# YuvalNirkin/hyperseg

Measured on AMD Instinct MI355X. Metric: frames/sec @ bs=1 HyperSeg-M 1024x512, higher is better.
Workload: dtype f32 storage and accumulation; level-4 inverted residual products as 3-term f16 splits (f32-class: 1.3e-7 of sum|a||b|; exact_f32 beside it)

## Files before the change

### hyperseg_amd/_hip.py

```python
import ctypes as C
import os
import types

import torch

_LIB_PATH = os.environ.get('HS_HIP_LIB') or os.path.join(os.path.dirname(os.path.abspath(__file__)), 'lib',
                                                         'libhyperseg_hip.so')

ACT_NONE, ACT_RELU, ACT_RELU6, ACT_SWISH = 0, 1, 2, 3
PAD_MODES = {'zeros': 0, 'reflect': 1, 'replicate': 2, 'circular': 3}
PREV_NONE, PREV_SAME, PREV_BILINEAR = 0, 1, 2

_STATUS = {-1: 'bad argument', -2: 'feature map does not tile into the weight grid (H % fh or W % fw != 0)',
           -3: 'unsupported shape', -4: 'tile does not fit the LDS'}


class HipLibraryError(RuntimeError):
    pass


class StageInputC(C.Structure):
    _fields_ = [('skip', C.c_void_p), ('prev', C.c_void_p),
                ('batch', C.c_int32), ('H', C.c_int32), ('W', C.c_int32),
                ('c_skip', C.c_int32), ('c_prev', C.c_int32),
# ... 15 lines not shown
    _fields_ = [('skip', C.c_void_p), ('c_skip', C.c_int32), ('bank', C.c_void_p), ('ld', C.c_int64), ('c_out', C.c_int32),
                ('scale', C.c_void_p), ('shift', C.c_void_p), ('act', C.c_int32)]


class SeTailC(C.Structure):
    _fields_ = [('w_reduce', C.c_void_p), ('b_reduce', C.c_void_p), ('w_expand_t', C.c_void_p), ('b_expand', C.c_void_p), ('c_squeezed', C.c_int32),
                ('gate', C.c_void_p), ('squeezed', C.c_void_p), ('workspace', C.c_void_p)]


class ChainIrLevelC(C.Structure):
    _fields_ = [('skip', C.c_void_p), ('c_skip', C.c_int32), ('bank', C.c_void_p), ('ld', C.c_int64), ('hidden', C.c_int32), ('c_out', C.c_int32),
                ('s1', C.c_void_p), ('b1', C.c_void_p), ('s2', C.c_void_p), ('b2', C.c_void_p), ('s3', C.c_void_p), ('b3', C.c_void_p)]


class S2wTrainLayerC(C.Structure):
    _fields_ = [('signal_index', C.c_int32), ('signal_channels', C.c_int32), ('groups', C.c_int32),
                ('w', C.c_void_p), ('wc', C.c_int32), ('rows', C.c_int32),
                ('bank', C.c_void_p), ('ld', C.c_int64), ('dbank', C.c_void_p), ('dw', C.c_void_p), ('ds', C.c_void_p)]


class TtaPassC(C.Structure):
    _fields_ = [('x', C.c_void_p), ('Hi', C.c_int32), ('Wi', C.c_int32), ('Hm', C.c_int32), ('Wm', C.c_int32),
                ('flipped', C.c_int32), ('entry', C.c_int32)]


STATUS = 'hs_status'
i32, i64, vp = C.c_int32, C.c_int64, C.c_void_p
SIGNATURES = {
    'hs_version': ([], C.c_int),
    'hs_build_info': ([], C.c_char_p),
    'hs_signal2weights_fwd': ([vp, i32, i32, i32, i32, i32, i32, i32, vp, i32, i32, vp, i64, vp], STATUS),
    'hs_signal2weights_multi_fwd': ([vp, i32, i32, i32, i32, C.POINTER(S2wLayerC), i32, vp], STATUS),
    'hs_s2w_pack_floats': ([i32, i32, i32], C.c_int64),
    'hs_s2w_pack_fwd': ([vp, i32, i32, i32, vp, vp], STATUS),
    'hs_bank_pack_fwd': ([vp, i32, i32, i32, i32, i32, i32, vp, i64, vp], STATUS),
    'hs_bn_fold_fwd': ([vp, vp, vp, vp, C.c_float, i32, vp, vp, vp], STATUS),
    'hs_patch_conv_fwd': ([C.POINTER(StageInputC), i32, i32, vp, i64, i32, i32, i32, i32, i32,
                           C.POINTER(EpilogueC), vp, vp], STATUS),
    'hs_patch_conv_s2w_fwd': ([C.POINTER(StageInputC), i32, i32, vp, i64, i32, i32, C.POINTER(EpilogueC), vp,
                               vp, i32, i32, i32, i32, C.POINTER(S2wLayerC), i32, vp], STATUS),
    'hs_k1_chain_workspace': ([i32, i32, i32, C.POINTER(K1LevelC), i32], C.c_int64),
    'hs_k1_chain_fwd': ([i32, i32, i32, C.POINTER(K1LevelC), i32, vp, vp, vp], STATUS),
    'hs_decoder_chain_workspace': ([i32, i32, i32, C.POINTER(K1LevelC), i32, C.POINTER(ChainIrLevelC)], C.c_int64),
    'hs_decoder_chain_fwd': ([i32, i32, i32, C.POINTER(K1LevelC), i32, C.POINTER(ChainIrLevelC), vp, vp, vp], STATUS),
    'hs_meta_conv_fwd': ([vp, i32, i32, i32, i32, vp, i64] + [i32] * 13 + [C.POINTER(EpilogueC), vp, vp], STATUS),
    'hs_meta_conv_bwd': ([vp, i32, i32, i32, i32, vp, i64] + [i32] * 12 + [vp, vp, vp, i64, vp], STATUS),
# ... 102 lines not shown
    'hs_label_resize_fwd': ([vp, i32, i32, i32, i32, vp, i32, vp, i32, i32, i32, i32, i32, i32, i32, vp, i32, vp], STATUS),
    'hs_resize_tables_fwd': ([vp, i32, i32, i32, i32, i32, i32, i32, vp, vp, vp, vp, vp], STATUS),
    'hs_frame_resize_batch_fwd': ([vp, i32, i32, i32, i32, vp, vp, vp, vp, i32, i32, i32, C.c_uint32, vp, vp, vp], STATUS),
    'hs_label_resize_batch_fwd': ([vp, i32, i32, i32, i32, vp, vp, vp, i32, i32, i32, vp, i32, vp], STATUS),
    'hs_label_encode_fwd': ([vp, i32, i32, i32, i32, vp, i32, i32, i32, vp, i32, vp], STATUS),
    'hs_label_resize_coded_fwd': ([vp, i32, i32, i32, i32, vp, i32, vp, i32, i32, i32, i32, i32, i32, i32, vp, i32, i32, i32, vp, i32, vp], STATUS),
    'hs_label_resize_batch_coded_fwd': ([vp, i32, i32, i32, i32, vp, vp, vp, i32, i32, i32, vp, i32, i32, i32, vp, i32, vp], STATUS),
    'hs_color_jitter_fwd': ([vp, i32, i32, i32, i32, vp, vp, vp, vp, vp], STATUS),
    'hs_gaussian_blur_fwd': ([vp, i32, i32, i32, i32, vp, vp, vp, vp, vp, vp], STATUS),
    'hs_frame_rotate_fwd': ([vp, i32, i32, i32, i32, vp, i32, i32, C.c_uint32, C.c_uint32, vp, vp, vp], STATUS),
    'hs_label_rotate_fwd': ([vp, i32, i32, i32, i32, vp, i32, i32, i32, i32, vp, i32, vp], STATUS),
    'hs_resize_tables_ragged_fwd': ([vp, i32, i32, i32, i32, i32, i32, i32, vp, vp, vp, vp, vp], STATUS),
    'hs_color_jitter_ragged_fwd': ([vp, i32, i32, i32, i32, vp, vp, vp, vp, vp], STATUS),
    'hs_frame_resize_ragged_fwd': ([vp, i32, i32, i32, i32, vp, vp, vp, vp, i32, i32, i32, vp, vp], STATUS),
    'hs_label_resize_ragged_fwd': ([vp, i32, i32, i32, i32, vp, vp, vp, i32, i32, vp, vp], STATUS),
    'hs_frame_rotate_ragged_fwd': ([vp, i32, i32, i32, i32, vp, vp, vp, i32, i32, C.c_uint32, C.c_uint32, vp, vp, vp], STATUS),
    'hs_label_rotate_ragged_fwd': ([vp, i32, i32, i32, vp, vp, vp, i32, i32, i32, i32, vp, i32, vp], STATUS),
    'hs_mbconv_expand_dw_fwd': ([vp, i32, i32, i32, i32, vp, i32, vp, vp, vp, i32, i32, i32, i32, i32, i32, vp, vp, vp, vp, vp], STATUS),
    'hs_se_gate_fwd': ([vp, i32, i32, i32, C.c_float, vp, vp, i32, vp, vp, vp, vp, vp, i32, vp, vp, vp], STATUS),
    'hs_gemm_split_kp': ([i32], C.c_int),
    'hs_gemm_split_fwd': ([vp, vp, vp, vp, vp, i32, vp, vp, i32, i32, i32, i32, i32, vp], STATUS),
    'hs_gemm_split_se_fwd': ([vp, vp, vp, i32, C.c_float, vp, vp, i32, vp, vp, vp, vp, i32, vp, vp, i32, i32, i32, i32, i32, vp, vp, vp], STATUS),
    'hs_gemm_split_se_route': ([i32] * 6, C.c_int),
    'hs_gemm_split_conv2x2_fwd': ([vp, vp, vp, vp, i32, vp, vp, i32, i32, i32, i32, i32, i32, vp], STATUS),
    'hs_gemm_split_up2_fwd': ([vp, vp, vp, vp, i32, vp, i32, i32, i32, i32, i32, i32, vp], STATUS),
    'hs_depthwise_route': ([i32] * 11, C.c_int),
    'hs_mbconv_route': ([i32] * 11, C.c_int),
    'hs_stem_dw_route': ([i32] * 9, C.c_int),
    'hs_stem_route': ([i32] * 3, C.c_int),
    'hs_se_gate_route': ([i32] * 5, C.c_int),
    'hs_pointwise_route': ([i32] * 5, C.c_int),
    'hs_pooled_shift_fwd': ([vp, i32, C.c_float, vp, vp, vp, i32, i32, vp], STATUS),
}
EXPORTS = list(SIGNATURES)


def check(status, what):
    if status == 0:
        return
    if status < 0:
        raise HipLibraryError(f'{what}: {_STATUS.get(status, status)}')
    raise HipLibraryError(f'{what}: HIP launch failed with hipError_t {status}')


def _raise_unless_ok(status, fn, args):
    if status:
# ... 65 lines not shown
```

### hyperseg_amd/csrc/hs_gemm_split.hip

```cpp
#include "hs_common.h"
#include "hs_se_gate_phases.h"
#include <type_traits>

namespace hs {

using half8 = __attribute__((ext_vector_type(8))) _Float16;
using gs_f32x4 = __attribute__((ext_vector_type(4))) float;

__device__ __forceinline__ int gs_exp_of(float m) { return min(max(__float_as_int(m) >> 23, 27), 254); }
__device__ __forceinline__ float gs_scale_of(int eb) { return __int_as_float((268 - eb) << 23); }
__device__ __forceinline__ float gs_inv_scale_of(int eb) { return __int_as_float((eb - 14) << 23); }

struct GemmSplitArgs {
    const _Float16* __restrict__ wf;
    const float* __restrict__ w_inv;
    const float* __restrict__ gate; const float* __restrict__ x;
    const float* shift;
    const float* residual;
    float* y;
    int M, K, KST, N, act;
    int conv_wo;
    float* pool_partial;
    int up2_wo;
};

struct GemmSeArgs {
    const float* __restrict__ partial;
    const float* __restrict__ w1; const float* __restrict__ b1;
    const float* __restrict__ w2t; const float* __restrict__ b2;
    float* gate_out; float* squeezed_out;
    float inv_hw; int nblk, Csq;
};
template <bool SEG> struct GemmSeOperand {};
template <> struct GemmSeOperand<true> : GemmSeArgs {};

#ifndef HS_GS_NARROW_MAX_WG
#define HS_GS_NARROW_MAX_WG 128
#endif

#ifndef HS_GS_TALL_MIN_WG
#define HS_GS_TALL_MIN_WG 257
#endif

template <int KS, int NWV, bool FAST, int NS, int MT, int NCH, bool PATCH, bool SEG = false>
__global__ __launch_bounds__(64 * NWV)
void gemm_split_kernel(GemmSplitArgs a, GemmSeOperand<SEG> se) {
    static_assert(!SEG || (FAST && !PATCH && NCH == 1 && (NWV == 8 ? KS <= 3 : KS == 1)), "SEG: the project convolutions' forms only");
    extern __shared__ __attribute__((aligned(16))) float gs_red[];
    constexpr int nthr = 64 * NWV, nwv = NWV;
    constexpr int NP = 16 * NS, NR = 16 * MT, NE = NR * NP;
    const int tid = threadIdx.x, lane = tid & 63, wave = tid >> 6;
    const int lrow = lane & 15, kg = lane >> 4;
    const int n0 = blockIdx.x * NP, r0 = blockIdx.y * MT, b = blockIdx.z;
    const float* __restrict__ xb = a.x + (size_t)b * a.K * a.N;
    const float* __restrict__ gb = a.gate ? a.gate + (size_t)b * a.K : nullptr;
    float* yb = a.y + (size_t)b * a.M * a.N * (a.up2_wo > 0 ? 4 : 1);
    const float* rb = a.residual ? a.residual + (size_t)b * a.M * a.N : nullptr;
    const int rt_max = (a.M + 15) >> 4;

    using gs_f32x2 = __attribute__((ext_vector_type(2))) float;
    const int ncol0 = min(n0 + NS * lrow, a.N - (FAST && !PATCH && NS == 2 ? 2 : 1)), ncol1 = min(n0 + NS * lrow + 1, a.N - 1);
    float xv[NCH][NS][KS][8];
    if constexpr (PATCH) {
        const int oy = ncol0 / a.conv_wo, ox = ncol0 - oy * a.conv_wo;
        const float* __restrict__ win = xb + (size_t)(2 * oy) * (2 * a.conv_wo) + 2 * ox;
        const int cmax = (a.K >> 2) - 1;
#pragma unroll
        for (int c = 0; c < NCH; ++c)
#pragma unroll
            for (int s = 0; s < KS; ++s)
#pragma unroll
                for (int q = 0; q < 4; ++q) {
                    const int ch = min((((wave * NCH + c) * KS + s) * 32 + 8 * kg) / 4 + (q >> 1), cmax);
                    const float* src = win + (size_t)ch * (4 * a.N) + (q & 1) * (2 * a.conv_wo);
                    if constexpr (NS == 1) {
                        const gs_f32x2 v = *reinterpret_cast<const gs_f32x2*>(src);
// ... 375 lines not shown
    GemmSeOperand<true> se{{partial, w_reduce, b_reduce, w_expand_t, b_expand, gate_out, squeezed_out, inv_hw, nblk, c_squeezed}};
    const size_t se_lds = (size_t)SEP_LDS_FLOATS * sizeof(float);
    const size_t lds = pol.lds > se_lds ? pol.lds : se_lds;
    hipStream_t s = (hipStream_t)stream;
#define HS_GSE(KSV, NWV) do { \
        if (pol.narrow) hipLaunchKernelGGL((gemm_split_kernel<KSV, NWV, true, 1, 2, 1, false, true>), pol.grid, dim3(64 * NWV), lds, s, a, se); \
        else if (pol.tall) hipLaunchKernelGGL((gemm_split_kernel<KSV, NWV, true, 2, 4, 1, false, true>), pol.grid, dim3(64 * NWV), lds, s, a, se); \
        else hipLaunchKernelGGL((gemm_split_kernel<KSV, NWV, true, 2, 2, 1, false, true>), pol.grid, dim3(64 * NWV), lds, s, a, se); } while (0)
    switch (pol.ks) {
        case 1: if (pol.nwv == 2) HS_GSE(1, 2); else if (pol.nwv == 4) HS_GSE(1, 4); else HS_GSE(1, 8); break;
        case 2: HS_GSE(2, 8); break;
        default: HS_GSE(3, 8); break;
    }
#undef HS_GSE
    return launch_status();
}

extern "C" int hs_gemm_split_fwd(const void* w_frag, const float* w_inv, const float* gate, const float* x,
                                 const float* shift, int32_t act, const float* residual, float* y,
                                 int32_t batch, int32_t c_out, int32_t c_in, int32_t kp, int32_t pixels, void* stream) {
    return launch_gemm_split_plain(w_frag, w_inv, gate, x, shift, act, residual, y, batch, c_out, c_in, kp, pixels, 0, stream);
}

extern "C" int hs_gemm_split_up2_fwd(const void* w_frag, const float* w_inv, const float* x, const float* shift, int32_t act,
                                     float* y, int32_t batch, int32_t c_out, int32_t c_in, int32_t kp, int32_t Ho, int32_t Wo,
                                     void* stream) {
    if (Ho <= 0 || Wo <= 0 || (((size_t)y) & 7) != 0) return HS_ERR_BAD_ARG;
    return launch_gemm_split_plain(w_frag, w_inv, nullptr, x, shift, act, nullptr, y, batch, c_out, c_in, kp, Ho * Wo, Wo, stream);
}

extern "C" int hs_pooled_shift_fwd(const float* partial, int32_t nblk, float inv_pixels, const float* wb, const float* shift,
                                   float* shift_out, int32_t rows, int32_t channels, void* stream) {
    if (!partial || !wb || !shift || !shift_out || nblk <= 0 || rows <= 0 || channels <= 0) return HS_ERR_BAD_ARG;
    if (channels > 8192) return HS_ERR_UNSUPPORTED;
    hipLaunchKernelGGL(pooled_shift_kernel, dim3((rows + 15) / 16), dim3(256), (size_t)channels * sizeof(float), (hipStream_t)stream,
                       partial, nblk, inv_pixels, wb, shift, shift_out, rows, channels);
    return launch_status();
}

extern "C" int hs_gemm_split_conv2x2_fwd(const void* w_frag, const float* w_inv, const float* x, const float* shift, int32_t act,
                                         float* y, float* pool_partial, int32_t batch, int32_t c_out, int32_t c_in, int32_t kp,
                                         int32_t Ho, int32_t Wo, void* stream) {
    if (!w_frag || !w_inv || !x || !y || batch <= 0 || c_out <= 0 || c_in <= 0 || Ho <= 0 || Wo <= 0) return HS_ERR_BAD_ARG;
    if (act < 0 || act > 3) return HS_ERR_BAD_ARG;
    int nwv, ks, nch;
    if (c_in > (1 << 20) || !gemm_split_plan(4 * c_in, nwv, ks, nch) || nwv != 8 || (Wo & 1) || (c_in & 1)) return HS_ERR_UNSUPPORTED;
// ... 24 lines not shown
```

### hyperseg_amd/functional.py

```python
import collections
import ctypes as C
import functools
import os
import threading

import torch

from . import _hip
from ._hip import ACT_NONE, ACT_RELU, ACT_RELU6, PAD_MODES

BN_EPS_DEFAULT = 1e-5
DTYPE_CODES = {torch.float32: 0, torch.bfloat16: 1, torch.float16: 2}
S2W_TRAIN_MAX_LAYERS = 8
COSCHEDULE_BANKS = os.environ.get('HS_COSCHEDULE_BANKS', '0') == '1'


def _round_up(n, m):
    return (n + m - 1) // m * m


def _device_of(a):
    if isinstance(a, torch.Tensor):
        return a.device
    if isinstance(a, (StageInput, BankRef, SignalRef, U8Frame)):
# ... 1111 lines not shown
def gemm_split(sw, x, gate=None, shift=None, act=ACT_NONE, residual=None, out=None):
    b, cin, h, w = x.shape
    if cin != sw.c_in:
        raise ValueError(f'input has {cin} channels, the weight {sw.c_in}')
    shape = (b, sw.c_out, h, w)
    if out is None:
        out = torch.empty(shape, device=x.device, dtype=torch.float32)
    elif tuple(out.shape) != shape:
        raise ValueError(f'out has shape {tuple(out.shape)}, expected {shape}')
    if residual is not None and tuple(residual.shape) != shape:
        raise ValueError(f'residual has shape {tuple(residual.shape)}, expected {shape}')
    if gate is not None and tuple(gate.shape) != (b, cin):
        raise ValueError(f'gate has shape {tuple(gate.shape)}, expected {(b, cin)}')
    if shift is not None and shift.numel() != sw.c_out:
        raise ValueError(f'shift has {shift.numel()} entries, expected {sw.c_out}')
    _hip.run.hs_gemm_split_fwd(_hip.dev_ptr(sw.frag, 'w_frag', torch.float16), _hip.dev_ptr(sw.inv, 'w_inv'),
                               _hip.dev_ptr(gate, 'gate') if gate is not None else None, _hip.dev_ptr(x, 'x'),
                               _hip.dev_ptr(shift, 'shift') if shift is not None else None, int(act),
                               _hip.dev_ptr(residual, 'residual') if residual is not None else None,
                               _hip.dev_ptr(out, 'out'), b, sw.c_out, cin, sw.kp, h * w, _hip.stream_ptr())
    return out


def gemm_split_se_route(channels, nblk, c_squeezed, c_out, pixels, aligned=True):
    r = _route(_hip.lib.hs_gemm_split_se_route(channels, nblk, c_squeezed, c_out, pixels, int(bool(aligned))), 'hs_gemm_split_se_route')
    return None if r is None else f'ks{r >> 4}_w{r & 15}'


@_on_operand_device
def gemm_split_se(sw, x, partial, hw, w_reduce, b_reduce, w_expand_t, b_expand, shift=None, act=ACT_NONE, residual=None, out=None,
                  gate_out=None, squeezed_out=None):
    b, cin, h, w = x.shape
    if cin != sw.c_in:
        raise ValueError(f'input has {cin} channels, the weight {sw.c_in}')
    shape = (b, sw.c_out, h, w)
    if out is None:
        out = torch.empty(shape, device=x.device, dtype=torch.float32)
    elif tuple(out.shape) != shape:
        raise ValueError(f'out has shape {tuple(out.shape)}, expected {shape}')
    if residual is not None and tuple(residual.shape) != shape:
        raise ValueError(f'residual has shape {tuple(residual.shape)}, expected {shape}')
    if shift is not None and shift.numel() != sw.c_out:
        raise ValueError(f'shift has {shift.numel()} entries, expected {sw.c_out}')
    if partial.dim() != 2 or partial.shape[0] != b * cin:
        raise ValueError(f'partial has shape {tuple(partial.shape)}, expected ({b * cin}, nblk)')
    csq = w_reduce.shape[0]
# ... 1074 lines not shown
```

### hyperseg_amd/models/backbones/efficientnet.py

```python
import math
from functools import partial

import torch
import torch.nn as nn
import torch.nn.functional as F

_B0_STAGES = [
    (1, 3, 1, 32, 16, 1),
    (6, 3, 2, 16, 24, 2),
    (6, 5, 2, 24, 40, 2),
    (6, 3, 2, 40, 80, 3),
    (6, 5, 1, 80, 112, 3),
    (6, 5, 2, 112, 192, 4),
    (6, 3, 1, 192, 320, 1),
]
_SCALING = {
    'efficientnet-b0': (1.0, 1.0, 224, 0.2), 'efficientnet-b1': (1.0, 1.1, 240, 0.2),
    'efficientnet-b2': (1.1, 1.2, 260, 0.3), 'efficientnet-b3': (1.2, 1.4, 300, 0.3),
    'efficientnet-b4': (1.4, 1.8, 380, 0.4), 'efficientnet-b5': (1.6, 2.2, 456, 0.4),
    'efficientnet-b6': (1.8, 2.6, 528, 0.5), 'efficientnet-b7': (2.0, 3.1, 600, 0.5),
}
_BN_MOMENTUM, _BN_EPS, _SE_RATIO, _DIVISOR = 0.01, 1e-3, 0.25, 8


# ... 112 lines not shown
                    size = _out_size(size, stride)
        self._res_feat_mask[-1] = True
        self.feat_channels = [c for c, m in zip(feat_nc, self._res_feat_mask) if m]

        if out_feat_scale is not None:
            for i, in_nc in enumerate(self.feat_channels):
                scale = out_feat_scale[i] if isinstance(out_feat_scale, (list, tuple)) else out_feat_scale
                out_nc = int(round(in_nc * scale))
                if scale != 1.:
                    self.add_module(f'_feat_fc_{i}', nn.Sequential(
                        SamePadConv2d(in_nc, out_nc, 1, image_size=res, bias=False), bn(out_nc)))
                else:
                    setattr(self, f'_feat_fc_{i}', None)
                self.feat_channels[i] = out_nc

        head_nc = round_filters(1280, width)
        self.feat_channels.append(head_nc)
        self._conv_head = SamePadConv2d(feat_nc[-1], head_nc, 1, image_size=size, bias=False)
        self._bn1 = bn(head_nc)
        self._avg_pooling = nn.AdaptiveAvgPool2d(1)
        self._dropout = nn.Dropout(dropout)
        self._fc = head(head_nc, num_classes) if head is not None else None
        self._fused_head, self._fused_fc, self._fused_stem = None, None, None

    def _fused_ok(self, inputs):
        if self._fused_stem is None and self._fused_head is None and all(b._fused_dw is None for b in self._blocks):
            return False
        if not _inference_only(self, inputs):
            return False
        h, w = (inputs.shape[2] + 1) // 2, (inputs.shape[3] + 1) // 2
        for blk in self._blocks:
            st = blk._depthwise_conv.stride[0]
            if (h * w) % 4 != 0:
                return False
            h, w = (h + st - 1) // st, (w + st - 1) // st
        return (h * w) % 4 == 0

    def takes_u8_frame(self, frame):
        f0 = self._blocks[0]._fused_dw if len(self._blocks) else None
        return self._fused_stem is not None and f0 is not None and f0.takes_image() and self._fused_ok(frame)

    def extract_features_list(self, inputs):
        use = self._fused_ok(inputs)
        for blk in self._blocks:
            blk._fused_active = use
        try:
            return self._extract_features_list(inputs, use)
        finally:
            for blk in self._blocks:
                blk._fused_active = None

    def _extract_features_list(self, inputs, use):
        f0 = self._blocks[0]._fused_dw if len(self._blocks) else None
        if self._fused_stem is not None and use and f0 is not None and getattr(f0, '_stem', None) is not None:
            x = inputs
        elif self._fused_stem is not None and use:
            x = self._fused_stem(inputs)
        else:
            x = F.silu(self._bn0(self._conv_stem(inputs)))
        feats = []
        n = len(self._blocks)
        for idx, block in enumerate(self._blocks):
            rate = self.drop_connect_rate * float(idx) / n if self.drop_connect_rate else None
            x = block(x, drop_connect_rate=rate)
            if self._res_feat_mask[idx]:
                fc = getattr(self, f'_feat_fc_{len(feats)}', None) if self.out_feat_scale is not None else None
                fused = self._fused_fc is not None and use and str(len(feats)) in self._fused_fc
                feats.append(self._fused_fc[str(len(feats))](x) if fused else (x if fc is None else fc(x)))
        if self._fused_head is not None and use:
            x = self._fused_head(x)
        else:
            x = F.silu(self._bn1(self._conv_head(x)))
        if self.pool:
            x = self._avg_pooling(x).flatten(1)
        x = self._dropout(x)
        if self._fc is not None:
            x = self._fc(x)
        feats.append(x)
        return feats

    def forward(self, inputs):
        feats = self.extract_features_list(inputs)
        return feats if self.return_features else feats[-1]


def efficientnet(model_name, pretrained=False, head=nn.Linear, **kwargs):
    if pretrained:
        raise RuntimeError('pretrained ImageNet weights need network access; load a checkpoint with '
                           'load_state_dict instead (parameter names match the reference)')
    return EfficientNet(model_name, head=head, **kwargs)
```

### hyperseg_amd/utils/inference.py

```python
import contextlib
import os

import torch
import torch.nn as nn

from ..models._common import Blend, Epilogue, HyperGenBase, Score


class InputNorm:

    LAYOUTS = ('hwc', 'chw')

    def __init__(self, mean=(0.485, 0.456, 0.406), std=(0.229, 0.224, 0.225), layout='hwc'):
        if layout not in self.LAYOUTS:
            raise ValueError(f'layout {layout!r}: expected one of {self.LAYOUTS}')
        self.mean = torch.as_tensor(mean, dtype=torch.float32).flatten().clone()
        self.std = torch.as_tensor(std, dtype=torch.float32).flatten().clone()
        if self.mean.numel() != 3 or self.std.numel() != 3:
            raise ValueError('mean and std must hold one value per channel of a 3-channel frame')
        if bool((self.std == 0).any()):
            raise ValueError('std must be non-zero')
        self.layout = layout
        values = torch.arange(256, dtype=torch.float32)
        self._tables = {torch.device('cpu'): ((values.div(255)[None, :] - self.mean[:, None]) / self.std[:, None]).contiguous()}
# ... 173 lines not shown

def _fold_sequential(seq):
    n = 0
    mods = list(seq)
    for i in range(len(mods) - 1):
        if isinstance(mods[i], nn.Conv2d) and isinstance(mods[i + 1], nn.BatchNorm2d) and not mods[i + 1].training:
            _fold(mods[i], mods[i + 1])
            seq[i + 1] = nn.Identity()
            n += 1
    return n


def _bn_affine(bn):
    with torch.no_grad():
        scale = bn.weight / torch.sqrt(bn.running_var + bn.eps)
        shift = bn.bias - bn.running_mean * scale
    return scale.detach().clone(), shift.detach().clone()


SPLIT_GEMM_MAX_K = int(os.environ.get('HS_SPLIT_GEMM_MAX_K', '1280'))
STEM_DW = os.environ.get('HS_STEM_DW', '1') != '0'
HS_GEMM_SE = os.environ.get('HS_GEMM_SE', '1') != '0'
GEMM_SE_MAX_CIN = 512
FUSE_EXPAND_MIN_PIXELS = int(os.environ.get('HS_FUSE_EXPAND_MIN_PIXELS', '2048'))
FUSE_EXPAND_MAX_CIN = int(os.environ.get('HS_FUSE_EXPAND_MAX_CIN', '40'))


LEAN_MFMA_MAX_CIN = int(os.environ.get('HS_LEAN_MFMA_MAX_CIN', '16'))
PW_MFMA_MAX_CIN = int(os.environ.get('HS_PW_MFMA_MAX_CIN', '96'))
PW_MFMA_MIN_PIXELS = int(os.environ.get('HS_PW_MFMA_MIN_PIXELS', '8192'))
GEMM_LT_MIN_PIXELS = int(os.environ.get('HS_GEMM_LT_MIN_PIXELS', '16384'))


@contextlib.contextmanager
def gemm_library(pixels, batch=1):
    want = os.environ.get('HS_BLAS') or ('cublaslt' if (pixels >= GEMM_LT_MIN_PIXELS or batch > 1) else 'cublas')
    prev = torch.backends.cuda.preferred_blas_library()
    torch.backends.cuda.preferred_blas_library(want)
    try:
        yield
    finally:
        torch.backends.cuda.preferred_blas_library(prev)


class FusedPointwise(nn.Module):

# ... 47 lines not shown
        with gemm_library(h * w, b):
            if b == 1:
                return torch.mm(self.conv.weight.view(-1, cin), x.view(cin, h * w)).view(1, -1, h, w)
            return torch.bmm(self.conv.weight.view(1, -1, cin).expand(b, -1, -1), x.view(b, cin, h * w)).view(b, -1, h, w)

    def forward(self, x, gate=None, residual=None):
        import torch.nn.functional as F
        from .. import functional as HF
        conv = self.conv
        x = x.contiguous()
        b, cin, h, w = x.shape
        if self.uses_mfma(x):
            return HF.pointwise_conv(x, conv.weight, gate, self.scale, self.shift, self.act, residual)
        if (h * w) % 4 != 0:
            raise NotImplementedError('feature maps with H*W % 4 != 0')
        sw = self.split_weights(True, x.device) if self.split_gemm else None
        if sw is not None:
            return HF.gemm_split(sw, x, gate=gate, shift=self.shift, act=self.act, residual=residual)
        if gate is None:
            y = F.conv2d(x, conv.weight) if b == 1 else self.raw(x)
        else:
            y = F.conv2d(x * gate[:, :, None, None], conv.weight)
        return HF.affine_act_(y, self.scale, self.shift, self.act, residual)


class FusedStem(nn.Module):

    def __init__(self, conv, bn):
        super().__init__()
        assert conv.kernel_size == (3, 3) and conv.stride == (2, 2) and conv.in_channels == 3 and conv.bias is None
        scale, shift = _bn_affine(bn)
        self.register_buffer('scale', scale, persistent=False)
        self.register_buffer('shift', shift, persistent=False)
        self._conv = [conv]
        if conv._pad is not None:
            self.pad_l, self.pad_t = conv._pad[0], conv._pad[2]
            self.pad_w, self.pad_h = conv._pad[0] + conv._pad[1], conv._pad[2] + conv._pad[3]
        else:
            self.pad_t, self.pad_l = conv.padding
            self.pad_h, self.pad_w = 2 * conv.padding[0], 2 * conv.padding[1]
        with torch.no_grad():
            self.register_buffer('w28', nn.functional.pad(conv.weight.detach().flatten(1), (0, 1)).contiguous(), persistent=False)

    def out_size(self, x):
        h, w = x.shape[2:]
        return (h + self.pad_h - 3) // 2 + 1, (w + self.pad_w - 3) // 2 + 1
# ... 23 lines not shown
            self.pad_h, self.pad_w = 2 * conv.padding[0], 2 * conv.padding[1]
        self.skip = blk.stride == 1 and blk.in_f == blk.out_f
        self._exp_t = None
        self._red_w = None
        self.se_tail = True
        self._stem = None
        if in_offset is not None:
            assert self.expand is not None, 'a depthwise conv cannot consume an offset tensor (zero padding)'
            self.expand.absorb_input_offset(in_offset)
        with torch.no_grad():
            carried = self.project.shift.clone()
            if self.skip and in_offset is not None:
                carried += in_offset.to(carried.device)
            self.defer_shift = bool(defer_shift)
            self.out_offset = carried.clone() if defer_shift else None
            self.project.shift.copy_(torch.zeros_like(carried) if defer_shift else carried)

    def takes_image(self):
        return self._stem is not None and STEM_DW

    def fuses_expand(self, x, ho, wo):
        return self.expand is not None and x.shape[1] <= FUSE_EXPAND_MAX_CIN and ho * wo >= FUSE_EXPAND_MIN_PIXELS

    def forward(self, inputs, blk):
        from .. import functional as HF
        pre = None
        if self._stem is not None and inputs.shape[1] == 3:
            stem = self._stem[0]
            img = inputs.contiguous()
            pre = HF.stem_dw(img, stem.w28, stem.scale, stem.shift, stem.pad_t, stem.pad_l, stem.out_size(img),
                             blk._depthwise_conv.weight, self.pad_t, self.pad_l, self.scale, self.shift, pool=True) if STEM_DW else None
            if pre is None and isinstance(img, HF.U8Frame):
                img = img.float_image()
            inputs = pre[0] if pre is not None else stem(img)
        x = inputs.contiguous()
        b, _, h, w = x.shape
        ho = (h + self.pad_h - self.k) // self.stride + 1
        wo = (w + self.pad_w - self.k) // self.stride + 1
        lean = True
        red, exp = blk._se_reduce, blk._se_expand
        if self._exp_t is None or self._exp_t.device != x.device:
            self._exp_t = exp.weight.detach().flatten(1).t().contiguous()
        if self._red_w is None or self._red_w.device != x.device:
            self._red_w = red.weight.detach().flatten(1)
        proj = self.project
        cmid = blk._depthwise_conv.weight.shape[0]
        lean_gemm = lean and (cmid > LEAN_MFMA_MAX_CIN if self.defer_shift else not proj.mfma_covers(cmid, ho * wo))
        folds = lean_gemm and not (proj.split_gemm and proj.split_weights(True, x.device) is not None)
        se = (self._red_w, red.bias, self._exp_t, exp.bias) if self.se_tail and not folds else None
        if pre is not None:
            out = (pre[0], pre[1], False) if se is not None else pre
        elif self.fuses_expand(x, ho, wo):
            out = HF.mbconv_expand_dw(x, self.expand.conv.weight, self.expand.scale, self.expand.shift,
                                      blk._depthwise_conv.weight, self.stride, self.pad_t, self.pad_l, (ho, wo),
                                      self.scale, self.shift, pool=True, se=se)
        else:
            in_scale = in_shift = None
            if self.expand is not None:
                if lean and not self.expand.uses_mfma(x):
                    in_scale, in_shift = self.expand.scale, self.expand.shift
                    x = self.expand.raw(x)
                else:
                    x = self.expand(x)
            out = HF.depthwise_conv_bn_act(x, blk._depthwise_conv.weight, self.stride, self.pad_t, self.pad_l,
                                           (ho, wo), self.scale, self.shift, act=3, pool=True,
                                           in_scale=in_scale, in_shift=in_shift, se=se)
        y, pooled, gated = out if se is not None else (out[0], out[1], False)

        def se_gate(**fold):
            if gated and not fold:
                return pooled
            return HF.se_gate(pooled, b, ho * wo, red.weight, red.bias, self._exp_t, exp.bias, **fold)
        skip = inputs.contiguous() if self.skip else None
        if lean_gemm:
            sw = proj.split_weights(True, y.device) if proj.split_gemm else None
            if sw is not None:
                if (HS_GEMM_SE and y.is_cuda and not gated and cmid <= GEMM_SE_MAX_CIN and
                        HF.gemm_split_se_route(cmid, pooled.shape[1], self._red_w.shape[0], sw.c_out, ho * wo,
                                               aligned=(pooled.data_ptr() | red.weight.data_ptr()) % 16 == 0) is not None):
                    se_ops = (pooled, ho * wo, red.weight, red.bias, self._exp_t, exp.bias)
                    if self.defer_shift:
                        if skip is None:
                            return HF.gemm_split_se(sw, y, *se_ops)
                        return HF.gemm_split_se(sw, y, *se_ops, residual=skip, out=skip)
# ... 113 lines not shown
                if pool is not None:
                    shift = HF.pooled_shift(pool, t.shape[2] * t.shape[3], self.wb_scaled, shift)
                else:
                    shift = torch.addmv(shift, self.wb_scaled, t.mean((2, 3)).view(half))
                sw_up = self._split_weights(f'up{level}', wgt[:, :half], scale) if self.split_gemm and (sh * sw) % 4 == 0 else None
                if sw_up is not None and level == 0:
                    HF.gemm_split_up2(sw_up, skip.contiguous(), shift=shift, act=HF.ACT_RELU, out=signal[:, half:])
                    return signal
                if sw_up is not None:
                    y = HF.gemm_split(sw_up, skip.contiguous(), shift=shift, act=HF.ACT_RELU)
                else:
                    y = HF.affine_act_(torch.mm(wgt[:, :half], skip.view(half, sh * sw)).view(1, half, sh, sw), scale, shift, HF.ACT_RELU)
                pooled_const = False
            else:
                y = torch.mm(wgt, torch.cat((skip, t), dim=1).view(cin, sh * sw)).view(1, half, sh, sw)
                y = HF.affine_act_(y, scale, shift, HF.ACT_RELU)
            if level > 0:
                t = wm.upsample(y)
            else:
                signal[:, half:].view(half, sh, 2, sw, 2).copy_(y.view(half, sh, 1, sw, 1).expand(half, sh, 2, sw, 2))
        return signal


def _fuse_backbone(bb):
    blocks = list(bb._blocks)
    offset, tap = None, 0
    bb._fused_fc = nn.ModuleDict()
    for idx, blk in enumerate(blocks):
        conv = blk._depthwise_conv
        ok = conv.kernel_size[0] in (3, 5) and conv.stride[0] in (1, 2) and isinstance(blk._bn1, nn.BatchNorm2d)
        tapped = bb._res_feat_mask[idx]
        fc = getattr(bb, f'_feat_fc_{tap}', None) if (tapped and bb.out_feat_scale is not None) else None
        if ok:
            nxt = blocks[idx + 1] if idx + 1 < len(blocks) else None
            nxt_ok = nxt is None or (nxt.expand != 1 and nxt._depthwise_conv.kernel_size[0] in (3, 5)
                                     and isinstance(nxt._bn1, nn.BatchNorm2d))
            defer = nxt_ok and (not tapped or isinstance(fc, nn.Sequential))
            blk._fused_dw = FusedMBConv(blk, in_offset=offset, defer_shift=defer)
            offset = blk._fused_dw.out_offset
        else:
            assert offset is None
        if tapped:
            if isinstance(fc, nn.Sequential):
                fused = FusedPointwise(fc[0], fc[1], act=0)
                if offset is not None:
                    fused.absorb_input_offset(offset)
                bb._fused_fc[str(tap)] = fused
            else:
                assert offset is None
            tap += 1
    stem = bb._conv_stem
    if stem.kernel_size == (3, 3) and stem.stride == (2, 2) and stem.in_channels == 3 and isinstance(bb._bn0, nn.BatchNorm2d):
        bb._fused_stem = FusedStem(stem, bb._bn0)
        f0 = blocks[0]._fused_dw if blocks else None
        if f0 is not None and f0.expand is None and f0.k == 3 and f0.stride == 1 and not f0.skip:
            f0._stem = [bb._fused_stem]
    bb._fused_head = FusedPointwise(bb._conv_head, bb._bn1, act=3)
    if offset is not None:
        bb._fused_head.absorb_input_offset(offset)


def _install_fused(model):
    bb, wm = model.backbone, model.weight_mapper
    for blk in bb._blocks:
        blk._fused_dw = None
    bb._fused_stem = bb._fused_head = bb._fused_fc = None
    _fuse_backbone(bb)
    dev = next(model.parameters()).device
    bb.to(dev)
    if type(wm).__name__ == 'WeightMapper' and hasattr(wm, 'in_conv') and hasattr(wm, 'up_blocks') and wm.levels >= 2:
        wm._fused = FusedContextHead(wm).to(dev)
        wm._fused.split_gemm = bool(getattr(model, '_hs_split_gemm', False))
    for m in bb.modules():
# ... 319 lines not shown
```

### include/hyperseg_hip.h

```cpp
#ifndef HYPERSEG_HIP_H
#define HYPERSEG_HIP_H

#include <stdint.h>

#ifdef __cplusplus
extern "C" {
#endif

#define HS_ABI_VERSION 1

typedef enum {
    HS_OK = 0,
    HS_ERR_BAD_ARG = -1,
    HS_ERR_NOT_DIVISIBLE = -2,
    HS_ERR_UNSUPPORTED = -3,
    HS_ERR_LDS = -4
} hs_status;

typedef enum { HS_ACT_NONE = 0, HS_ACT_RELU = 1, HS_ACT_RELU6 = 2, HS_ACT_SWISH = 3 } hs_act;
typedef enum { HS_PAD_ZEROS = 0, HS_PAD_REFLECT = 1, HS_PAD_REPLICATE = 2, HS_PAD_CIRCULAR = 3 } hs_pad_mode;
typedef enum { HS_PREV_NONE = 0, HS_PREV_SAME = 1, HS_PREV_BILINEAR = 2 } hs_prev_mode;

typedef struct {
    const float* skip;
// ... 370 lines not shown
int hs_mbconv_route(int32_t batch, int32_t c_in, int32_t H, int32_t W, int32_t c_mid, int32_t k, int32_t stride,
                    int32_t Ho, int32_t Wo, int32_t aligned16, int32_t with_se_tail);
int hs_stem_dw_route(int32_t H, int32_t W, int32_t c_mid, int32_t stem_pad_t, int32_t stem_pad_l, int32_t Hs, int32_t Ws,
                     int32_t k, int32_t aligned16);
#define HS_SE_ROUTE_FUSED 0
#define HS_SE_ROUTE_EARLY 1
#define HS_SE_ROUTE_FUSED_WIDE 2
#define HS_SE_ROUTE_TWO_LAUNCH 3
int hs_se_gate_route(int32_t channels, int32_t nblk, int32_t c_squeezed, int32_t with_w_proj, int32_t aligned16);
#define HS_PW_ROUTE(nb, nt, vec) (((nb) << 8) | ((nt) << 4) | (vec))
int hs_pointwise_route(int32_t batch, int32_t c_in, int32_t c_out, int32_t pixels, int32_t aligned16);

int hs_gemm_split_kp(int32_t c_in);
int hs_gemm_split_fwd(const void* w_frag, const float* w_inv, const float* gate, const float* x, const float* shift,
                      int32_t act, const float* residual, float* y, int32_t batch, int32_t c_out, int32_t c_in, int32_t kp,
                      int32_t pixels, void* stream);
#define HS_GSE_ROUTE(ks, nwv) (((ks) << 4) | (nwv))
int hs_gemm_split_se_fwd(const void* w_frag, const float* w_inv, const float* partial, int32_t nblk, float inv_hw,
                         const float* w_reduce, const float* b_reduce, int32_t c_squeezed, const float* w_expand_t,
                         const float* b_expand, const float* x, const float* shift, int32_t act, const float* residual,
                         float* y, int32_t batch, int32_t c_out, int32_t c_in, int32_t kp, int32_t pixels,
                         float* gate_out, float* squeezed_out, void* stream);
int hs_gemm_split_se_route(int32_t channels, int32_t nblk, int32_t c_squeezed, int32_t c_out, int32_t pixels, int32_t aligned16);
int hs_gemm_split_conv2x2_fwd(const void* w_frag, const float* w_inv, const float* x, const float* shift, int32_t act, float* y,
                              float* pool_partial, int32_t batch, int32_t c_out, int32_t c_in, int32_t kp, int32_t Ho,
                              int32_t Wo, void* stream);
int hs_gemm_split_up2_fwd(const void* w_frag, const float* w_inv, const float* x, const float* shift, int32_t act, float* y,
                          int32_t batch, int32_t c_out, int32_t c_in, int32_t kp, int32_t Ho, int32_t Wo, void* stream);
int hs_pooled_shift_fwd(const float* partial, int32_t nblk, float inv_pixels, const float* wb, const float* shift,
                        float* shift_out, int32_t rows, int32_t channels, void* stream);

int hs_halo_tiles_fwd(int32_t dtype, const void* x, int32_t batch, int32_t channels, int32_t H, int32_t W, int32_t fh, int32_t fw,
                      void* tiled, int32_t patch_major, void* stream);
int hs_halo_tiles_bwd(int32_t dtype, const void* dtiled, int32_t batch, int32_t channels, int32_t H, int32_t W, int32_t fh, int32_t fw,
                      void* dx, int32_t patch_major, void* stream);
int hs_tile_interior_fwd(int32_t dtype, const void* tiled, int32_t batch, int32_t channels, int32_t H, int32_t W, int32_t fh,
                         int32_t fw, void* y, void* stream);
int hs_tile_interior_bwd(int32_t dtype, const void* dy, int32_t batch, int32_t channels, int32_t H, int32_t W, int32_t fh, int32_t fw,
                         void* dtiled, void* stream);
int hs_dw_tiles_fwd(int32_t dtype, const void* tiled, const float* bank, int64_t ld, int32_t batch, int32_t channels, int32_t H, int32_t W,
                    int32_t fh, int32_t fw, void* y, int32_t patch_major, void* stream);
int hs_dw_tiles_bwd_in(int32_t dtype, const void* dy, const float* bank, int64_t ld, int32_t batch, int32_t channels, int32_t H, int32_t W,
                       int32_t fh, int32_t fw, void* dtiled, int32_t patch_major, void* stream);
int hs_dw_tiles_bwd_w(int32_t dtype, const void* tiled, const void* dy, int32_t batch, int32_t channels, int32_t H, int32_t W, int32_t fh,
                      int32_t fw, float* dbank, int64_t ld, int32_t patch_major, void* stream);
int64_t hs_bootstrap_mean_workspace(void);
// ... 104 lines not shown
```

Before: 1371.

## Pair feature-tap 1x1 conv with next block's expand GEMM in one launch

Adds a paired split-f16 GEMM kernel. Blocks along grid.y are split between two weight problems that share the same input tensor, so a backbone feature-tap projection and the following block's expand conv (or the head conv) run in a single launch. The backbone records which tap each following block hosts and defers the tap into that block's expand or the head. This saves a kernel launch and a separate read of the input per tap, at the cost of more dispatch conditions and fallbacks when routes or shapes do not match.

```diff
diff --git a/hyperseg_amd/_hip.py b/hyperseg_amd/_hip.py
--- a/hyperseg_amd/_hip.py
+++ b/hyperseg_amd/_hip.py
@@ -61,6 +61,11 @@
 class TtaPassC(C.Structure):
     _fields_ = [('x', C.c_void_p), ('Hi', C.c_int32), ('Wi', C.c_int32), ('Hm', C.c_int32), ('Wm', C.c_int32),
                 ('flipped', C.c_int32), ('entry', C.c_int32)]
+
+
+class GemmSplitProblemC(C.Structure):
+    _fields_ = [('w_frag', C.c_void_p), ('w_inv', C.c_void_p), ('shift', C.c_void_p), ('y', C.c_void_p),
+                ('act', C.c_int32), ('c_out', C.c_int32), ('c_in', C.c_int32), ('kp', C.c_int32)]
 
 
 STATUS = 'hs_status'
@@ -209,6 +214,8 @@
     'hs_gemm_split_fwd': ([vp, vp, vp, vp, vp, i32, vp, vp, i32, i32, i32, i32, i32, vp], STATUS),
     'hs_gemm_split_se_fwd': ([vp, vp, vp, i32, C.c_float, vp, vp, i32, vp, vp, vp, vp, i32, vp, vp, i32, i32, i32, i32, i32, vp, vp, vp], STATUS),
     'hs_gemm_split_se_route': ([i32] * 6, C.c_int),
+    'hs_gemm_split_pair_fwd': ([C.POINTER(GemmSplitProblemC), C.POINTER(GemmSplitProblemC), vp, vp, vp, i32, i32, vp], STATUS),
+    'hs_gemm_split_pair_route': ([i32] * 8, C.c_int),
     'hs_gemm_split_conv2x2_fwd': ([vp, vp, vp, vp, i32, vp, vp, i32, i32, i32, i32, i32, i32, vp], STATUS),
     'hs_gemm_split_up2_fwd': ([vp, vp, vp, vp, i32, vp, i32, i32, i32, i32, i32, i32, vp], STATUS),
     'hs_depthwise_route': ([i32] * 11, C.c_int),
diff --git a/hyperseg_amd/csrc/hs_gemm_split.hip b/hyperseg_amd/csrc/hs_gemm_split.hip
--- a/hyperseg_amd/csrc/hs_gemm_split.hip
+++ b/hyperseg_amd/csrc/hs_gemm_split.hip
@@ -31,8 +31,14 @@
     float* gate_out; float* squeezed_out;
     float inv_hw; int nblk, Csq;
 };
-template <bool SEG> struct GemmSeOperand {};
-template <> struct GemmSeOperand<true> : GemmSeArgs {};
+struct GemmPairArgs {
+    const _Float16* __restrict__ wf; const float* __restrict__ w_inv;
+    const float* shift; float* y;
+    int M, act, ny1;
+};
+template <bool SEG, bool PAIR = false> struct GemmSeOperand {};
+template <> struct GemmSeOperand<true, false> : GemmSeArgs {};
+template <> struct GemmSeOperand<false, true> : GemmPairArgs {};
 
 #ifndef HS_GS_NARROW_MAX_WG
 #define HS_GS_NARROW_MAX_WG 128
@@ -42,16 +48,24 @@
 #define HS_GS_TALL_MIN_WG 257
 #endif
 
-template <int KS, int NWV, bool FAST, int NS, int MT, int NCH, bool PATCH, bool SEG = false>
+template <int KS, int NWV, bool FAST, int NS, int MT, int NCH, bool PATCH, bool SEG = false, bool PAIR = false>
 __global__ __launch_bounds__(64 * NWV)
-void gemm_split_kernel(GemmSplitArgs a, GemmSeOperand<SEG> se) {
+void gemm_split_kernel(GemmSplitArgs a, GemmSeOperand<SEG, PAIR> se) {
     static_assert(!SEG || (FAST && !PATCH && NCH == 1 && (NWV == 8 ? KS <= 3 : KS == 1)), "SEG: the project convolutions' forms only");
+    static_assert(!PAIR || (FAST && !SEG && !PATCH && NCH == 1), "PAIR: plain FAST single-chunk forms only");
     extern __shared__ __attribute__((aligned(16))) float gs_red[];
     constexpr int nthr = 64 * NWV, nwv = NWV;
     constexpr int NP = 16 * NS, NR = 16 * MT, NE = NR * NP;
     const int tid = threadIdx.x, lane = tid & 63, wave = tid >> 6;
     const int lrow = lane & 15, kg = lane >> 4;
-    const int n0 = blockIdx.x * NP, r0 = blockIdx.y * MT, b = blockIdx.z;
+    int by = blockIdx.y;
+    if constexpr (PAIR) {
+        if (by >= se.ny1) {
+            by -= se.ny1;
+            a.wf = se.wf; a.w_inv = se.w_inv; a.shift = se.shift; a.y = se.y; a.M = se.M; a.act = se.act;
+        }
+    }
+    const int n0 = blockIdx.x * NP, r0 = by * MT, b = blockIdx.z;
     const float* __restrict__ xb = a.x + (size_t)b * a.K * a.N;
     const float* __restrict__ gb = a.gate ? a.gate + (size_t)b * a.K : nullptr;
     float* yb = a.y + (size_t)b * a.M * a.N * (a.up2_wo > 0 ? 4 : 1);
@@ -473,6 +487,57 @@
     return launch_gemm_split_plain(w_frag, w_inv, gate, x, shift, act, residual, y, batch, c_out, c_in, kp, pixels, 0, stream);
 }
 
+static int gemm_split_pair_route(int batch, int c_out1, int c_in1, int c_out2, int c_in2, int pixels, bool gated, bool residual,
+                                 GemmSplitPolicy& pol, int& ny2) {
+    if (batch <= 0 || c_out1 <= 0 || c_in1 <= 0 || c_out2 <= 0 || c_in2 <= 0 || pixels <= 0) return HS_ERR_BAD_ARG;
+    if (gated || residual || c_in1 != c_in2) return HS_ERR_UNSUPPORTED;
+    const int kp = hs_gemm_split_kp(c_in1);
+    if (kp < 0) return HS_ERR_UNSUPPORTED;
+    const int pst = gemm_split_policy(batch, c_out1, c_in1, kp, pixels, pol);
+    if (pst != HS_OK) return pst;
+    if (pol.nch != 1 || !pol.fast) return HS_ERR_UNSUPPORTED;
+    const int mt = pol.tall ? 4 : 2;
+    ny2 = ((c_out2 + 15) / 16 + mt - 1) / mt;
+    if ((size_t)pol.grid.y + (size_t)ny2 > 65535) return HS_ERR_UNSUPPORTED;
+    return HS_GSP_ROUTE(pol.narrow ? HS_GSP_NARROW : pol.tall ? HS_GSP_TALL : HS_GSP_PLAIN, pol.ks, pol.nwv);
+}
+
+extern "C" int hs_gemm_split_pair_route(int32_t batch, int32_t c_out1, int32_t c_in1, int32_t c_out2, int32_t c_in2, int32_t pixels,
+                                        int32_t gated, int32_t residual) {
+    GemmSplitPolicy pol;
+    int ny2;
+    return gemm_split_pair_route(batch, c_out1, c_in1, c_out2, c_in2, pixels, gated != 0, residual != 0, pol, ny2);
+}
+
+extern "C" int hs_gemm_split_pair_fwd(const hs_gemm_split_problem* p1, const hs_gemm_split_problem* p2, const float* gate, const float* x,
+                                      const float* residual, int32_t batch, int32_t pixels, void* stream) {
+    if (!p1 || !p2 || !x) return HS_ERR_BAD_ARG;
+    if (!p1->w_frag || !p1->w_inv || !p1->y || !p2->w_frag || !p2->w_inv || !p2->y) return HS_ERR_BAD_ARG;
+    if (p1->act < 0 || p1->act > 3 || p2->act < 0 || p2->act > 3) return HS_ERR_BAD_ARG;
+    GemmSplitPolicy pol;
+    int ny2;
+    const int route = gemm_split_pair_route(batch, p1->c_out, p1->c_in, p2->c_out, p2->c_in, pixels, gate != nullptr, residual != nullptr, pol, ny2);
+    if (route < 0) return route;
+    if (p1->kp != pol.nwv * pol.ks * 32 || p2->kp != p1->kp) return HS_ERR_BAD_ARG;
+    GemmSplitArgs a{(const _Float16*)p1->w_frag, p1->w_inv, nullptr, x, p1->shift, nullptr, p1->y, p1->c_out, p1->c_in, p1->kp / 32, pixels, p1->act, 0, nullptr, 0};
+    GemmSeOperand<false, true> pr{{(const _Float16*)p2->w_frag, p2->w_inv, p2->shift, p2->y, p2->c_out, p2->act, (int)pol.grid.y}};
+    dim3 grid(pol.grid.x, pol.grid.y + ny2, pol.grid.z);
+    hipStream_t s = (hipStream_t)stream;
+#define HS_GPR(KSV, NWV) do { \
+        if (pol.narrow) hipLaunchKernelGGL((gemm_split_kernel<KSV, NWV, true, 1, 2, 1, false, false, true>), grid, dim3(64 * NWV), pol.lds, s, a, pr); \
+        else if (pol.tall) hipLaunchKernelGGL((gemm_split_kernel<KSV, NWV, true, 2, 4, 1, false, false, true>), grid, dim3(64 * NWV), pol.lds, s, a, pr); \
+        else hipLaunchKernelGGL((gemm_split_kernel<KSV, NWV, true, 2, 2, 1, false, false, true>), grid, dim3(64 * NWV), pol.lds, s, a, pr); } while (0)
+    switch (pol.ks) {
+        case 1: if (pol.nwv == 2) HS_GPR(1, 2); else if (pol.nwv == 4) HS_GPR(1, 4); else HS_GPR(1, 8); break;
+        case 2: HS_GPR(2, 8); break;
+        case 3: HS_GPR(3, 8); break;
+        case 4: HS_GPR(4, 8); break;
+        default: HS_GPR(5, 8); break;
+    }
+#undef HS_GPR
+    return launch_status();
+}
+
 extern "C" int hs_gemm_split_up2_fwd(const void* w_frag, const float* w_inv, const float* x, const float* shift, int32_t act,
                                      float* y, int32_t batch, int32_t c_out, int32_t c_in, int32_t kp, int32_t Ho, int32_t Wo,
                                      void* stream) {
diff --git a/hyperseg_amd/functional.py b/hyperseg_amd/functional.py
--- a/hyperseg_amd/functional.py
+++ b/hyperseg_amd/functional.py
@@ -1157,6 +1157,42 @@
     return out
 
 
+_GSP_FORMS = {0: 'plain', 1: 'narrow', 2: 'tall'}
+
+
+def gemm_split_pair_route(batch, c_out1, c_in1, c_out2, c_in2, pixels, gated=False, residual=False):
+    r = _route(_hip.lib.hs_gemm_split_pair_route(batch, c_out1, c_in1, c_out2, c_in2, pixels, int(bool(gated)), int(bool(residual))),
+               'hs_gemm_split_pair_route')
+    return None if r is None else f'{_GSP_FORMS[r >> 8]}_ks{(r >> 4) & 15}_w{r & 15}'
+
+
+def _gemm_split_problem(sw, shift, act, out):
+    return _hip.GemmSplitProblemC(_hip.dev_ptr(sw.frag, 'w_frag', torch.float16), _hip.dev_ptr(sw.inv, 'w_inv'),
+                                  _hip.dev_ptr(shift, 'shift') if shift is not None else None, _hip.dev_ptr(out, 'out'),
+                                  int(act), sw.c_out, sw.c_in, sw.kp)
+
+
+@_on_operand_device
+def gemm_split_pair(x, sw1, sw2, shift1=None, act1=ACT_NONE, shift2=None, act2=ACT_NONE, out1=None, out2=None, gate=None, residual=None):
+    b, cin, h, w = x.shape
+    if cin != sw1.c_in:
+        raise ValueError(f'input has {cin} channels, the first weight {sw1.c_in}')
+    outs = []
+    for sw, shift, out in ((sw1, shift1, out1), (sw2, shift2, out2)):
+        shape = (b, sw.c_out, h, w)
+        if out is None:
+            out = torch.empty(shape, device=x.device, dtype=torch.float32)
+        elif tuple(out.shape) != shape:
+            raise ValueError(f'out has shape {tuple(out.shape)}, expected {shape}')
+        if shift is not None and shift.numel() != sw.c_out:
+            raise ValueError(f'shift has {shift.numel()} entries, expected {sw.c_out}')
+        outs.append(out)
+    p1, p2 = _gemm_split_problem(sw1, shift1, act1, outs[0]), _gemm_split_problem(sw2, shift2, act2, outs[1])
+    _hip.run.hs_gemm_split_pair_fwd(C.byref(p1), C.byref(p2), _hip.dev_ptr(gate, 'gate') if gate is not None else None, _hip.dev_ptr(x, 'x'),
+                                    _hip.dev_ptr(residual, 'residual') if residual is not None else None, b, h * w, _hip.stream_ptr())
+    return outs[0], outs[1]
+
+
 def gemm_split_se_route(channels, nblk, c_squeezed, c_out, pixels, aligned=True):
     r = _route(_hip.lib.hs_gemm_split_se_route(channels, nblk, c_squeezed, c_out, pixels, int(bool(aligned))), 'hs_gemm_split_se_route')
     return None if r is None else f'ks{r >> 4}_w{r & 15}'
diff --git a/hyperseg_amd/models/backbones/efficientnet.py b/hyperseg_amd/models/backbones/efficientnet.py
--- a/hyperseg_amd/models/backbones/efficientnet.py
+++ b/hyperseg_amd/models/backbones/efficientnet.py
@@ -158,6 +158,7 @@
         self._dropout = nn.Dropout(dropout)
         self._fc = head(head_nc, num_classes) if head is not None else None
         self._fused_head, self._fused_fc, self._fused_stem = None, None, None
+        self._tap_host = None
 
     def _fused_ok(self, inputs):
         if self._fused_stem is None and self._fused_head is None and all(b._fused_dw is None for b in self._blocks):
@@ -196,14 +197,27 @@
             x = F.silu(self._bn0(self._conv_stem(inputs)))
         feats = []
         n = len(self._blocks)
+        hosts = (self._tap_host or {}) if use else {}
+        riding = None
         for idx, block in enumerate(self._blocks):
             rate = self.drop_connect_rate * float(idx) / n if self.drop_connect_rate else None
-            x = block(x, drop_connect_rate=rate)
+            if riding is not None:
+                x, feats[riding[0]] = block._fused_dw(x, block, tap=riding[1])
+                riding = None
+            else:
+                x = block(x, drop_connect_rate=rate)
             if self._res_feat_mask[idx]:
                 fc = getattr(self, f'_feat_fc_{len(feats)}', None) if self.out_feat_scale is not None else None
                 fused = self._fused_fc is not None and use and str(len(feats)) in self._fused_fc
-                feats.append(self._fused_fc[str(len(feats))](x) if fused else (x if fc is None else fc(x)))
-        if self._fused_head is not None and use:
+                host_on = self._fused_head is not None if idx + 1 == n else self._blocks[idx + 1]._fused_dw is not None
+                if fused and hosts.get(len(feats)) == idx + 1 and host_on:
+                    riding = (len(feats), self._fused_fc[str(len(feats))])
+                    feats.append(None)
+                else:
+                    feats.append(self._fused_fc[str(len(feats))](x) if fused else (x if fc is None else fc(x)))
+        if riding is not None:
+            x, feats[riding[0]] = self._fused_head.paired(x, riding[1])
+        elif self._fused_head is not None and use:
             x = self._fused_head(x)
         else:
             x = F.silu(self._bn1(self._conv_head(x)))
diff --git a/hyperseg_amd/utils/inference.py b/hyperseg_amd/utils/inference.py
--- a/hyperseg_amd/utils/inference.py
+++ b/hyperseg_amd/utils/inference.py
@@ -219,6 +219,7 @@
 STEM_DW = os.environ.get('HS_STEM_DW', '1') != '0'
 HS_GEMM_SE = os.environ.get('HS_GEMM_SE', '1') != '0'
 GEMM_SE_MAX_CIN = 512
+HS_TAP_PAIR = os.environ.get('HS_TAP_PAIR', '1') != '0'
 FUSE_EXPAND_MIN_PIXELS = int(os.environ.get('HS_FUSE_EXPAND_MIN_PIXELS', '2048'))
 FUSE_EXPAND_MAX_CIN = int(os.environ.get('HS_FUSE_EXPAND_MAX_CIN', '40'))
 
@@ -312,6 +313,20 @@
         else:
             y = F.conv2d(x * gate[:, :, None, None], conv.weight)
         return HF.affine_act_(y, self.scale, self.shift, self.act, residual)
+
+    def paired(self, x, tap, raw=False):
+        from .. import functional as HF
+        if (HS_TAP_PAIR and x.is_cuda and self.split_gemm and tap.split_gemm and not tap.uses_mfma(x)
+                and (raw or not self.uses_mfma(x)) and (x.shape[2] * x.shape[3]) % 4 == 0):
+            x = x.contiguous()
+            b, cin, h, w = x.shape
+            sw1, sw2 = self.split_weights(not raw, x.device), tap.split_weights(True, x.device)
+            if (sw1 is not None and sw2 is not None
+                    and HF.gemm_split_pair_route(b, sw1.c_out, sw1.c_in, sw2.c_out, sw2.c_in, h * w) is not None):
+                return HF.gemm_split_pair(x, sw1, sw2, shift1=None if raw else self.shift, act1=HF.ACT_NONE if raw else self.act,
+                                          shift2=tap.shift, act2=tap.act)
+        feat = tap(x)
+        return (self.raw(x) if raw else self(x)), feat
 
 
 class FusedStem(nn.Module):
@@ -381,7 +396,14 @@
     def fuses_expand(self, x, ho, wo):
         return self.expand is not None and x.shape[1] <= FUSE_EXPAND_MAX_CIN and ho * wo >= FUSE_EXPAND_MIN_PIXELS
 
-    def forward(self, inputs, blk):
+    def forward(self, inputs, blk, tap=None):
+        if tap is None:
+            return self._forward(inputs, blk, None, None)
+        feat = []
+        y = self._forward(inputs, blk, tap, feat)
+        return y, feat[0]
+
+    def _forward(self, inputs, blk, tap, feat):
         from .. import functional as HF
         pre = None
         if self._stem is not None and inputs.shape[1] == 3:
@@ -397,6 +419,10 @@
         ho = (h + self.pad_h - self.k) // self.stride + 1
         wo = (w + self.pad_w - self.k) // self.stride + 1
         lean = True
+        pairs = (tap is not None and pre is None and self.expand is not None and not self.fuses_expand(x, ho, wo)
+                 and not self.expand.uses_mfma(x))
+        if tap is not None and not pairs:
+            feat.append(tap(x))
         red, exp = blk._se_reduce, blk._se_expand
         if self._exp_t is None or self._exp_t.device != x.device:
             self._exp_t = exp.weight.detach().flatten(1).t().contiguous()
@@ -418,7 +444,11 @@
             if self.expand is not None:
                 if lean and not self.expand.uses_mfma(x):
                     in_scale, in_shift = self.expand.scale, self.expand.shift
-                    x = self.expand.raw(x)
+                    if pairs:
+                        x, f = self.expand.paired(x, tap, raw=True)
+                        feat.append(f)
+                    else:
+                        x = self.expand.raw(x)
                 else:
                     x = self.expand(x)
             out = HF.depthwise_conv_bn_act(x, blk._depthwise_conv.weight, self.stride, self.pad_t, self.pad_l,
@@ -578,10 +608,30 @@
         return signal
 
 
+def tap_pair_host(blocks, idx, host=None, launch='expand'):
+    n = len(blocks)
+    host = idx + 1 if host is None else host
+    if not idx < host <= n or launch not in ('expand', 'project', 'head') or (launch == 'head') != (host == n):
+        return None
+
+    def writes_input(b):
+        return b.stride == 1 and b.in_f == b.out_f
+
+    if any(writes_input(blocks[j]) for j in range(idx + 1, host)):
+        return None
+    if host < n:
+        if launch == 'project' and writes_input(blocks[host]):
+            return None
+        if launch == 'expand' and blocks[host].expand == 1:
+            return None
+    return host, launch
+
+
 def _fuse_backbone(bb):
     blocks = list(bb._blocks)
     offset, tap = None, 0
     bb._fused_fc = nn.ModuleDict()
+    bb._tap_host = {}
     for idx, blk in enumerate(blocks):
         conv = blk._depthwise_conv
         ok = conv.kernel_size[0] in (3, 5) and conv.stride[0] in (1, 2) and isinstance(blk._bn1, nn.BatchNorm2d)
@@ -602,9 +652,13 @@
                 if offset is not None:
                     fused.absorb_input_offset(offset)
                 bb._fused_fc[str(tap)] = fused
+                host = tap_pair_host(blocks, idx, launch='head' if idx + 1 == len(blocks) else 'expand')
+                if host is not None:
+                    bb._tap_host[tap] = host[0]
             else:
                 assert offset is None
             tap += 1
+    bb._tap_host = {t: h for t, h in bb._tap_host.items() if h == len(blocks) or blocks[h]._fused_dw is not None}
     stem = bb._conv_stem
     if stem.kernel_size == (3, 3) and stem.stride == (2, 2) and stem.in_channels == 3 and isinstance(bb._bn0, nn.BatchNorm2d):
         bb._fused_stem = FusedStem(stem, bb._bn0)
diff --git a/include/hyperseg_hip.h b/include/hyperseg_hip.h
--- a/include/hyperseg_hip.h
+++ b/include/hyperseg_hip.h
@@ -416,6 +416,18 @@
                          float* y, int32_t batch, int32_t c_out, int32_t c_in, int32_t kp, int32_t pixels,
                          float* gate_out, float* squeezed_out, void* stream);
 int hs_gemm_split_se_route(int32_t channels, int32_t nblk, int32_t c_squeezed, int32_t c_out, int32_t pixels, int32_t aligned16);
+typedef struct hs_gemm_split_problem {
+    const void* w_frag; const float* w_inv;
+    const float* shift;
+    float* y;
+    int32_t act, c_out, c_in, kp;
+} hs_gemm_split_problem;
+enum { HS_GSP_PLAIN = 0, HS_GSP_NARROW = 1, HS_GSP_TALL = 2 };
+#define HS_GSP_ROUTE(form, ks, nwv) (((form) << 8) | ((ks) << 4) | (nwv))
+int hs_gemm_split_pair_fwd(const hs_gemm_split_problem* p1, const hs_gemm_split_problem* p2, const float* gate, const float* x,
+                           const float* residual, int32_t batch, int32_t pixels, void* stream);
+int hs_gemm_split_pair_route(int32_t batch, int32_t c_out1, int32_t c_in1, int32_t c_out2, int32_t c_in2, int32_t pixels,
+                             int32_t gated, int32_t residual);
 int hs_gemm_split_conv2x2_fwd(const void* w_frag, const float* w_inv, const float* x, const float* shift, int32_t act, float* y,
                               float* pool_partial, int32_t batch, int32_t c_out, int32_t c_in, int32_t kp, int32_t Ho,
                               int32_t Wo, void* stream);
```

Result: no change. 1384 (median of 6 runs) (+0.9%).
